# Yaling-Li/DMA-YOLO

Measured on AMD Instinct MI355X. Metric: train images/sec (fwd+loss+bwd+optimizer, train.py batch loop) @1536; detect p50 ms incl. NMS, higher is better.
Workload: dtype bf16; 1 GPU; yolov5l-ca-sppfcspc-bifpn-scconv.yaml train @1536 nc=10; model=yolov5l-ca-sppfcspc-bifpn-scconv.yaml, global_batch=32, img=1536, parallelism=dp1

## Files before the change

dma-yolo_amd/csrc/bwd1x1.hip:

```cpp
#include "common.h"

namespace {
namespace b1 {

constexpr unsigned kOob = 0xFFFFFFF0u;

DEV __amdgpu_buffer_rsrc_t rsrc(const void* base, unsigned bytes) {
  return __builtin_amdgcn_make_buffer_rsrc(const_cast<void*>(base), 0, (int)bytes, 0x00020000);
}
DEV uint4 bload(__amdgpu_buffer_rsrc_t r, unsigned off) {
  const auto v = __builtin_amdgcn_raw_buffer_load_b128(r, off, 0, 0);
  return *reinterpret_cast<const uint4*>(&v);
}

template <int ROW> DEV int ksw(int k, int row) {
  constexpr int RB = ROW * 2;
  const int c = row >> 3, w = row & 7;
  int key;
  if constexpr (RB >= 256) key = 2 * ((k & 3) | (((k >> 3) & 1) << 2));
  else key = 2 * (((k >> 1) & 1) | (((k >> 3) & 1) << 1));
  return k * ROW + (((c ^ key) & (ROW / 8 - 1)) << 3) + w;
}
template <int K> DEV int wsw(int r, int ch) {
  if constexpr (K * 2 >= 256) return (ch ^ (r & 15)) & (K / 8 - 1);
  else return (ch ^ ((r >> 1) & 7)) & (K / 8 - 1);
}
template <int ROW> DEV bf16x8 frag_t(const bf16* base, int r0, int k0, int lane) {
  typedef short s4 __attribute__((ext_vector_type(4)));
  const int g = lane >> 4, il = lane & 15, q = il >> 2, p = il & 3;
  const bf16* a0 = base + ksw<ROW>(k0 + 8 * g + q, r0 + 4 * p);
  const bf16* a1 = base + ksw<ROW>(k0 + 8 * g + 4 + q, r0 + 4 * p);
  const s4 lo = __builtin_amdgcn_ds_read_tr16_b64_v4i16((__attribute__((address_space(3))) s4*)(a0));
  const s4 hi = __builtin_amdgcn_ds_read_tr16_b64_v4i16((__attribute__((address_space(3))) s4*)(a1));
  bf16x8 r;
  r[0] = lo[0]; r[1] = lo[1]; r[2] = lo[2]; r[3] = lo[3];
  r[4] = hi[0]; r[5] = hi[1]; r[6] = hi[2]; r[7] = hi[3];
  return r;
}
DEV unsigned pk2(float a, float b) {
  const bf16 x = __float2bfloat16(a), y = __float2bfloat16(b);
  return (unsigned)*reinterpret_cast<const unsigned short*>(&x) |
         ((unsigned)*reinterpret_cast<const unsigned short*>(&y) << 16);
}

template <int K, int CB, int TP, int PX>
struct Shape {
  static constexpr int NT = 256, KCH = K / 8, CCH = CB / 8;
  static constexpr int NDZ = TP * KCH / NT, NX = TP * CCH / NT;
  static constexpr int RDZ = NT / KCH, RXS = NT / CCH;
  static constexpr int KW = K / 2, CW = CB / 2, MI = KW / 16, NJ = CW / 16;
  static constexpr int PGN = TP / (16 * PX), U = PGN * (CB / 64), UPW = (U + 3) / 4;
  static constexpr int LDS = (CB * K + TP * K + TP * CB) * 2;
  static_assert(K % 64 == 0 && CB % 64 == 0 && NT % KCH == 0 && NT % CCH == 0, "channels");
  static_assert(NDZ >= 1 && NX >= 1 && TP % 32 == 0 && TP % (16 * PX) == 0 && U >= 1, "tile");
  static_assert(LDS <= 160 * 1024, "LDS");
};

template <int K, int CB, int TP, int PX>
__global__ void __launch_bounds__(256, 1) conv1x1_bwd_bn(
    const bf16* __restrict__ dy, long dps, const bf16* __restrict__ z, const bf16* __restrict__ x, long xps,
    const bf16* __restrict__ wt, const float* __restrict__ scale, const float* __restrict__ shift,
    const float* __restrict__ mean, const float* __restrict__ invstd, int act, const float* __restrict__ ca,
    const float* __restrict__ cb, const float* __restrict__ cc, bf16* __restrict__ dx, long bps, int accumulate,
    float* __restrict__ dw, float* __restrict__ dws, long M, int ntiles, int C, int nsplit, unsigned dyb, unsigned zb,
    unsigned xb) {
  using S = Shape<K, CB, TP, PX>;
  extern __shared__ __attribute__((aligned(16))) char b1_smem[];
  bf16* ws = reinterpret_cast<bf16*>(b1_smem);
  bf16* dzs = ws + CB * K;
  bf16* xs = dzs + TP * K;
  const int tid = threadIdx.x, lane = tid & 63, wid = tid >> 6, g = lane >> 4, il = lane & 15;
  const int slot = blockIdx.x >> 3, cs = slot % nsplit;
  const int grp = (blockIdx.x & 7) + 8 * (slot / nsplit), ngrp = gridDim.x / nsplit;
  const int cbase = cs * CB;
  x += cbase;
  dx += cbase;
  dw += cbase;

  for (int e = tid; e < CB * S::KCH; e += S::NT) {
    const int r = e / S::KCH, ch = e % S::KCH;
    *reinterpret_cast<uint4*>(ws + r * K + (wsw<K>(r, ch) << 3)) =
        *reinterpret_cast<const uint4*>(wt + (long)(cbase + r) * K + ch * 8);
  }

  const int kc8 = (tid % S::KCH) * 8, xc8 = (tid % S::CCH) * 8;
  float sc[8], sh[8], k1[8], k0[8], k2[8];
  {
    float t0[8], t1[8];
    ldf<8>(scale + kc8, sc);
    ldf<8>(shift + kc8, sh);
    ldf<8>(ca + kc8, k1);
    ldf<8>(cc + kc8, k2);
    ldf<8>(invstd + kc8, t0);
    ldf<8>(cb + kc8, k0);
    ldf<8>(mean + kc8, t1);
#pragma unroll
    for (int j = 0; j < 8; ++j) {
      k2[j] = k2[j] * t0[j];
      k0[j] = k0[j] - k2[j] * t1[j];
    }
  }

  const __amdgpu_buffer_rsrc_t rdy = rsrc(dy, dyb), rz = rsrc(z, zb), rx = rsrc(x, xb - 2u * cbase);
  uint4 pg[S::NDZ], pz[S::NDZ], pxv[S::NX];
  auto issue = [&](int t) {
    const long m0 = (long)t * TP;
#pragma unroll
    for (int j = 0; j < S::NDZ; ++j) {
      const long m = m0 + tid / S::KCH + j * S::RDZ;
      const bool ok = m < M;
      pg[j] = bload(rdy, ok ? (unsigned)((m * dps + kc8) * 2) : kOob);
      pz[j] = bload(rz, ok ? (unsigned)((m * K + kc8) * 2) : kOob);
    }
#pragma unroll
    for (int j = 0; j < S::NX; ++j) {
      const long m = m0 + tid / S::CCH + j * S::RXS;
      pxv[j] = bload(rx, m < M ? (unsigned)((m * xps + xc8) * 2) : kOob);
    }
  };

  f32x4 wacc[S::MI][S::NJ];
#pragma unroll
  for (int i = 0; i < S::MI; ++i)
#pragma unroll
    for (int j = 0; j < S::NJ; ++j) wacc[i][j] = f32x4{0.f, 0.f, 0.f, 0.f};
  const int wk = wid >> 1, wc = wid & 1;
  const int chq = (g & 1) * 16 + (g >> 1) * 8;

  int t = grp;
  if (t < ntiles) issue(t);
  __syncthreads();
  for (; t < ntiles; t += ngrp) {
    const long m0 = (long)t * TP;
#pragma unroll
    for (int j = 0; j < S::NDZ; ++j) {
      float zf[8], gf[8], o[8];
      unpack<bf16>(pz[j], zf);
      unpack<bf16>(pg[j], gf);
#pragma unroll
      for (int e = 0; e < 8; ++e) o[e] = zf[e] * sc[e] + sh[e];
      act_grad_n<8>(act, o);
#pragma unroll
      for (int e = 0; e < 8; ++e) o[e] = k1[e] * (gf[e] * o[e]) + k0[e] + k2[e] * zf[e];
      pg[j] = pack<bf16>(o);
    }
    __syncthreads();
#pragma unroll
    for (int j = 0; j < S::NDZ; ++j)
      *reinterpret_cast<uint4*>(dzs + ksw<K>(tid / S::KCH + j * S::RDZ, kc8)) = pg[j];
#pragma unroll
    for (int j = 0; j < S::NX; ++j)
      *reinterpret_cast<uint4*>(xs + ksw<CB>(tid / S::CCH + j * S::RXS, xc8)) = pxv[j];
    __syncthreads();

    uint4 old[S::UPW][PX][2];
    if (accumulate) {
#pragma unroll
      for (int s = 0; s < S::UPW; ++s) {
        const int u = wid + 4 * s, p0 = (u % S::PGN) * 16 * PX, c0 = (u / S::PGN) * 64;
        if (u >= S::U) break;
#pragma unroll
        for (int pt = 0; pt < PX; ++pt) {
          const long m = m0 + p0 + pt * 16 + il;
#pragma unroll
          for (int h = 0; h < 2; ++h)
            old[s][pt][h] = m < M ? *reinterpret_cast<const uint4*>(dx + m * bps + c0 + h * 32 + chq)
                                  : make_uint4(0, 0, 0, 0);
        }
      }
    }
    if (t + ngrp < ntiles) issue(t + ngrp);

#pragma unroll
    for (int s = 0; s < S::UPW; ++s) {
      const int u = wid + 4 * s, p0 = (u % S::PGN) * 16 * PX, c0 = (u / S::PGN) * 64;
      if (u >= S::U) break;
      f32x4 acc[4][PX];
#pragma unroll
      for (int ct = 0; ct < 4; ++ct)
#pragma unroll
        for (int pt = 0; pt < PX; ++pt) acc[ct][pt] = f32x4{0.f, 0.f, 0.f, 0.f};
#pragma unroll 2
// ... 22 lines not shown
          uint4 v;
          v.x = s0[0];
          v.y = s1[0];
          v.z = s0[1];
          v.w = s1[1];
          if (accumulate) {
            float f[8], o[8];
            unpack<bf16>(v, f);
            unpack<bf16>(old[s][pt][h], o);
#pragma unroll
            for (int j = 0; j < 8; ++j) f[j] += o[j];
            v = pack<bf16>(f);
          }
          if (m < M) *reinterpret_cast<uint4*>(dx + m * bps + c0 + h * 32 + chq) = v;
        }
      }
    }

#pragma unroll
    for (int ps = 0; ps < TP / 32; ++ps) {
      bf16x8 a[S::MI];
#pragma unroll
      for (int i = 0; i < S::MI; ++i) a[i] = frag_t<K>(dzs, wk * S::KW + i * 16, ps * 32, lane);
#pragma unroll
      for (int j = 0; j < S::NJ; ++j) {
        const bf16x8 b = frag_t<CB>(xs, wc * S::CW + j * 16, ps * 32, lane);
#pragma unroll
        for (int i = 0; i < S::MI; ++i)
          wacc[i][j] = __builtin_amdgcn_mfma_f32_16x16x32_bf16(a[i], b, wacc[i][j], 0, 0, 0);
      }
    }
  }
  float* part = dws != nullptr ? dws + (long)blockIdx.x * K * CB : nullptr;
#pragma unroll
  for (int i = 0; i < S::MI; ++i)
#pragma unroll
    for (int j = 0; j < S::NJ; ++j)
#pragma unroll
      for (int r = 0; r < 4; ++r) {
        const int kk = wk * S::KW + i * 16 + 4 * g + r, c = wc * S::CW + j * 16 + il;
        if (part != nullptr) part[kk * CB + c] = wacc[i][j][r];
        else atomicAdd(dw + (long)kk * C + c, wacc[i][j][r]);
      }
}

__global__ void __launch_bounds__(256) wgrad_slots_reduce(const float* __restrict__ dws, float* __restrict__ dw, int K,
                                                          int C, int CB, int nblocks, int nsplit) {
  const long e = (long)blockIdx.x * blockDim.x + threadIdx.x;
  if (e >= (long)K * C) return;
  const int k = (int)(e / C), c = (int)(e % C), cs = c / CB, cl = c % CB;
  float s = 0.f;
  for (int b = 0; b < nblocks; ++b)
    if (((b >> 3) % nsplit) == cs) s += dws[((long)b * K + k) * CB + cl];
  dw[e] += s;
}

int num_cus() {
  static int n = 0;
  if (n == 0) {
    int dev = 0;
    (void)hipGetDevice(&dev);
    if (hipDeviceGetAttribute(&n, hipDeviceAttributeMultiprocessorCount, dev) != hipSuccess || n <= 0) n = 256;
  }
  return n;
}

struct Plan {
  int cb, tp, px;
};
constexpr Plan plan(int K, int C) {
  return (K == 64 && C == 64) ? Plan{64, 128, 2} : (K == 128 && C == 64) ? Plan{64, 128, 2}
       : (K == 64 && C == 128) ? Plan{128, 64, 2} : (K == 128 && C == 128) ? Plan{128, 64, 2}
       : (K == 128 && C == 256) ? Plan{256, 64, 2} : (K == 128 && C == 512) ? Plan{256, 64, 2}
       : (K == 256 && C == 256) ? Plan{128, 32, 1} : (K == 256 && C == 128) ? Plan{128, 32, 1}
       : (K == 64 && C == 256) ? Plan{256, 64, 2} : Plan{0, 0, 0};
}

inline int grid_blocks(long M, int K, int C) {
  const Plan pl = plan(K, C);
  const int ns = C / pl.cb, ntiles = ceil_div(M, pl.tp);
  int ngrp = num_cus() / ns;
  if (ngrp > ntiles) ngrp = (ntiles + 7) / 8 * 8;
  return ngrp * ns;
}

template <int K, int C>
int launch(const bf16* dy, long dps, const bf16* z, const bf16* x, long xps, const bf16* wt, const float* scale,
           const float* shift, const float* mean, const float* invstd, int act, const float* ca, const float* cb,
           const float* cc, bf16* dx, long bps, int acc, float* dw, float* ws, long M, hipStream_t st) {
  constexpr Plan pl = plan(K, C);
  constexpr int CB = pl.cb, TP = pl.tp, PX = pl.px, NS = C / CB;
  using S = Shape<K, CB, TP, PX>;
  static bool raised = false;
  if (!raised) {
    (void)hipFuncSetAttribute((const void*)conv1x1_bwd_bn<K, CB, TP, PX>,
                              hipFuncAttributeMaxDynamicSharedMemorySize, S::LDS);
    raised = true;
  }
  const int nb = grid_blocks(M, K, C);
  conv1x1_bwd_bn<K, CB, TP, PX><<<nb, 256, S::LDS, st>>>(
      dy, dps, z, x, xps, wt, scale, shift, mean, invstd, act, ca, cb, cc, dx, bps, acc, dw, ws, M, ceil_div(M, TP), C,
      NS, (unsigned)(2.0 * (double)M * dps), (unsigned)(2.0 * (double)M * K), (unsigned)(2.0 * (double)M * xps));
  if (ws != nullptr)
    wgrad_slots_reduce<<<ceil_div((long)K * C, 256), 256, 0, st>>>(ws, dw, K, C, CB, nb, NS);
  return (int)hipGetLastError();
}
}
}

DMY_API int dmy_conv1x1_bwd_bn_ok(long M, int K, int C, long dps, long xps, long bps, const void* dy, const void* z,
                                  const void* x, const void* dx) {
  if (b1::plan(K, C).cb == 0 || M <= 0) return 0;
  if (dps % 8 || xps % 8 || bps % 8 || dps < K || xps < C || bps < C) return 0;
  for (const void* p : {dy, z, x, dx})
    if (((uintptr_t)p & 15) != 0) return 0;
  const double lim = (double)b1::kOob - 64.0;
  if (2.0 * (double)M * dps >= lim || 2.0 * (double)M * K >= lim || 2.0 * (double)M * xps >= lim) return 0;
  return 1;
}

DMY_API long dmy_conv1x1_bwd_bn_ws_elems(long M, int K, int C) {
  if (b1::plan(K, C).cb == 0 || M <= 0) return 0;
  return (long)b1::grid_blocks(M, K, C) * K * b1::plan(K, C).cb;
}

DMY_API int dmy_conv1x1_bwd_bn(const void* dy, long dps, const void* z, const void* x, long xps, const void* wt,
                               const float* scale, const float* shift, const float* mean, const float* invstd, int act,
                               const float* ca, const float* cb, const float* cc, void* dx, long bps, int accumulate,
                               float* dw, float* ws, long ws_elems, long M, int K, int C, void* stream) {
  if (!dmy_conv1x1_bwd_bn_ok(M, K, C, dps, xps, bps, dy, z, x, dx)) return -1;
  if (ws != nullptr && ws_elems < dmy_conv1x1_bwd_bn_ws_elems(M, K, C)) return -1;
  hipStream_t st = (hipStream_t)stream;
#define B1_GO(K_, C_)                                                                                                 \
  if (K == K_ && C == C_)                                                                                            \
    return b1::launch<K_, C_>((const bf16*)dy, dps, (const bf16*)z, (const bf16*)x, xps, (const bf16*)wt, scale,     \
                              shift, mean, invstd, act, ca, cb, cc, (bf16*)dx, bps, accumulate, dw, ws, M, st);
  B1_GO(64, 64)
  B1_GO(128, 64)
  B1_GO(64, 128)
  B1_GO(128, 128)
  B1_GO(128, 256)
  B1_GO(128, 512)
  B1_GO(256, 128)
  B1_GO(256, 256)
  B1_GO(64, 256)
#undef B1_GO
  return -1;
}
```

dma-yolo_amd/dmayolo/_lib.py:

```python
import ctypes
import os

import torch

_HERE = os.path.dirname(os.path.abspath(__file__))
LIB_PATH = os.path.join(_HERE, 'libdmayolo_hip.so')
if os.environ.get('DMY_LIB_AB'):
    LIB_PATH = os.path.join(_HERE, os.path.basename(os.environ['DMY_LIB_AB']))

P, I, L, F, D = ctypes.c_void_p, ctypes.c_int, ctypes.c_long, ctypes.c_float, ctypes.c_double

SIGNATURES = {
    'dmy_conv_fwd_partial_rows': [L, I],
    'dmy_conv_fwd_bound_rows': [L, I],
    'dmy_conv_fwd_last_rows': [],
    'dmy_conv_fwd_bn_rows': [I, P, P, P, P, I, I, I, I, L, I, I, I, I, I, I, I, L],
    'dmy_conv_fwd': [I, P, P, P, P, P, P, I, I, I, I, L, I, I, I, I, I, I, I, L, P],
    'dmy_conv_dgrad': [I, P, P, P, I, I, I, I, I, L, I, I, I, I, I, I, I, L, P],
    'dmy_conv_wgrad': [I, P, P, P, I, I, I, I, L, I, I, I, I, I, I, I, L, P],
    'dmy_conv_wprep_multi': [I, P, I, P],
    'dmy_conv_wprep_s2d': [I, P, P, I, I, I, P],
    'dmy_conv_wgrad_s2d_to_oihw': [P, P, I, I, I, P],
    'dmy_image_s2d': [I, I, P, P, I, I, I, I, I, F, P],
    'dmy_conv_fwd_act': [I, P, P, P, P, I, I, I, I, L, I, I, I, I, I, I, I, L, P, P, I, P, L, P],
    'dmy_conv_fwd_splitk_elems': [I, P, P, P, I, I, I, I, L, I, I, I, I, I, I, I, L],
    'dmy_conv_fwd_act_ws': [I, P, P, P, P, I, I, I, I, L, I, I, I, I, I, I, I, L, P, P, I, P, L, P, L, P],
    'dmy_conv_wgrad_ex': [I, P, P, P, I, I, I, I, L, I, I, I, I, I, I, I, L, I, P],
    'dmy_conv_wgrad_ws_elems': [I, P, P, I, I, I, I, L, I, I, I, I, I, I, I, L, I],
    'dmy_conv_wgrad_det': [I, P, P, P, I, I, I, I, L, I, I, I, I, I, I, I, L, I, P, L, P],
    'dmy_conv_route': [I, I, P, P, P, I, I, I, I, L, I, I, I, I, I, I, I, L, I],
    'dmy_conv_wprep': [I, P, P, P, I, I, I, I, I, P],
    'dmy_dwconv_ok': [I, P, P, P, I, I, I, I, I, I, L, I, I, I, I, I, I, L],
    'dmy_dwconv_fwd_rows': [L, I],
    'dmy_dwconv_fwd': [I, P, P, P, P, P, P, I, I, I, I, L, I, I, I, I, I, I, L, P],
    'dmy_dwconv_fwd_act': [I, P, P, P, P, I, I, I, I, L, I, I, I, I, I, I, L, P, P, I, P, L, P],
    'dmy_dwconv_dgrad': [I, P, P, P, I, I, I, I, I, L, I, I, I, I, I, I, L, P],
    'dmy_dwconv_wgrad_rows': [L, I],
    'dmy_dwconv_wgrad': [I, P, P, P, I, I, I, I, L, I, I, I, I, I, I, L, P],
    'dmy_dwconv_wgrad_finalize': [P, I, I, I, I, P, I, P],
    'dmy_conv1x1_bwd_bn_ok': [L, I, I, L, L, L, P, P, P, P],
    'dmy_conv1x1_bwd_bn': [P, L, P, P, L, P, P, P, P, P, I, P, P, P, P, L, I, P, P, L, L, I, I, P],
    'dmy_conv1x1_bwd_bn_ws_elems': [L, I, I],
    'dmy_aug_desc_bytes': [],
    'dmy_augment_batch': [P, I, P, I, I, P],
    'dmy_mosaic_desc_bytes': [],
    'dmy_mosaic_compose': [P, I, I, P],
    'dmy_fp8_quant_ws_elems': [],
    'dmy_fp8_quant': [P, L, I, L, P, P, P],
    'dmy_conv_wprep_fp8': [P, P, P, I, I, I, I, P],
    'dmy_conv_fwd_fp8_partial_rows': [L, I],
    'dmy_conv_fwd_fp8': [P, P, P, P, P, P, P, P, I, I, I, I, I, I, I, I, I, I, I, L, P, P, I, P, L, P],
    'dmy_conv_wgrad_to_oihw': [P, P, I, I, I, I, I, P],
    'dmy_bn_partial_rows': [L],
    'dmy_bn_stats': [I, P, L, L, I, P, P, P],
    'dmy_bn_finalize': [P, P, I, I, D, P, P, P, P, P, F, F, I, P, P, P, P, P],
    'dmy_bn_eval_coef': [P, P, P, P, F, I, P, P, P],
    'dmy_bn_act_fwd': [I, P, L, P, P, I, P, L, P, L, L, I, P],
    'dmy_bn_act_f8_blocks': [],
    'dmy_bn_act_fwd_f8': [P, L, P, P, I, P, L, P, L, L, I, P, P, P, P, F, P, P],
    'dmy_bn_bwd_reduce': [I, P, L, P, L, P, P, P, P, I, L, I, P, P, P],
    'dmy_bn_bwd_finalize': [P, P, I, I, D, P, P, P, P, P, P, P, P],
    'dmy_bn_bwd_apply': [I, P, L, P, L, P, P, P, P, I, P, P, P, P, L, L, I, P],
    'dmy_reduce_rows': [P, I, I, P, I, P],
    'dmy_bn_reduce_rows': [I, P, L, P, L, L, I],
    'dmy_colsum2_rows': [L],
    'dmy_colsum2': [P, P, L, I, P, P, P],
    'dmy_maxpool_fwd': [I, P, L, P, L, P, I, I, I, I, I, P],
    'dmy_maxpool_chain3_fwd': [I, P, L, P, P, P, L, I, I, I, I, I, P],
    'dmy_maxpool_bwd': [I, P, L, P, P, L, I, I, I, I, I, I, P],
    'dmy_avgpool_fwd': [I, P, L, P, I, I, I, I, I, P],
    'dmy_avgpool_bwd': [I, P, P, L, I, I, I, I, I, I, P],
    'dmy_resize_fwd': [I, P, L, P, L, F, I, I, I, I, I, I, P],
    'dmy_resize_bwd': [I, P, L, P, L, I, I, I, I, I, I, P],
    'dmy_slice_copy': [I, P, L, P, L, L, I, P, I, I, F, I, P],
    'dmy_slice_copy_dot': [I, P, L, P, L, P, L, L, I, P, I, I, F, I, P, P],
# ... 123 lines not shown
```

dma-yolo_amd/dmayolo/functional.py:

```python
import os
import weakref
from collections import namedtuple

import torch

from . import _lib
from ._lib import call, ptr, stream, ACT_NONE, ACT_SILU, ACT_HARDSWISH, ACT_SIGMOID, ACT_GELU, ACT_RELU

DT = {torch.float32: 0, torch.bfloat16: 1}
CL = torch.channels_last


def dcode(t):
    try:
        return DT[t.dtype]
    except KeyError:
        raise TypeError(f'dmayolo kernels take float32 or bfloat16 activations, got {t.dtype}')


def pixel_stride(t):
    N, C, H, W = t.shape
    for attempt in range(2):
        s = t.stride()
        if C == 1 or s[1] == 1:
# ... 518 lines not shown
    if OH < 1 or OW < 1 or C % VW[x.dtype] or p != k // 2 or k not in (3, 5) or s not in (1, 2):
        raise _dw_unsupported(G, C, K, k, s, p)
    g = ConvGeom(N, C, H, W, xps, K, k, s, p, OH, OW, N * OH * OW, C, H, W, k, s, p, C, 0, G)
    w = spec.wcache[1] if infer and spec.wcache is not None and spec.wcache[0] == wkey else None
    pre = WeightPrep.current.get(weight, x.dtype) if WeightPrep.current is not None else None
    if w is None and pre is not None:
        w = pre[1]
    elif w is None:
        w = prep_weight(weight, x.dtype, True)[1]
        if infer:
            spec.wcache = (wkey, w)
    return x, g, w, w, wkey


def _conv_fp8(x, g, weight, spec, wkey, f8in, prod, infer):
    if not (spec.fp8 and g.groups == 1 and not g.s2d and g.Cp == g.C and fp8_eligible(g.C, g.K, x.dtype, g.N * g.H * g.W)):
        return None
    if f8in is not None and (f8in[0].numel() != g.N * g.H * g.W * g.C or not F8_DELAYED[0]):
        f8in = None
    f8 = _fp8_operands(x, g.xps, weight, spec, wkey, f8in)
    if f8in is None and prod is not None and prod.f8_emit is None and F8_DELAYED[0] and not infer:
        prod.f8_emit = F8Emit(x.device)
    return f8


def _conv_infer(x, g, wf, bias, spec, res, rps, out, yps, f8):
    y = out if out is not None else new_act(g.N, g.K, g.OH, g.OW, x)
    scale, shift = eval_coef(spec, x.device) if spec.bn is not None else (None, None)
    epi = None if (scale is None and spec.act == ACT_NONE and res is None) else (scale, shift, spec.act, res, rps)
    _launch_conv_fwd(x, g, wf, bias, y, yps, None, None, epi=epi, f8=f8)
    return y


def _conv_bn_stats(x, g, wf, bias, z, bn, train_bn, f8):
    K, M, dev = g.K, g.M, x.device
    scale, shift, mean, invstd = f32(K, dev), f32(K, dev), f32(K, dev), f32(K, dev)
    if not train_bn:
        _launch_conv_fwd(x, g, wf, bias, z, K, None, None, f8=f8)
        call('dmy_bn_eval_coef', ptr(bn.weight), ptr(bn.bias), ptr(bn.running_mean), ptr(bn.running_var),
             float(bn.eps), K, ptr(scale), ptr(shift), stream())
        return scale, shift, mean, invstd
    dw = g.groups != 1
    P = call('dmy_dwconv_fwd_rows' if dw else 'dmy_conv_fwd_fp8_partial_rows' if f8 is not None else
             'dmy_conv_fwd_bound_rows', M, K)
    psum, psq = f32(P * K, dev), f32(P * K, dev)
    _launch_conv_fwd(x, g, wf, bias, z, K, psum, psq, f8=f8)
    if f8 is None and not dw:
        P = call('dmy_conv_fwd_last_rows')
    psum, psq, P = _fold_partials(psum, psq, P, K, dev)
    upd = int(bn.training and bn.track_running_stats)
    if upd:
        PARAM_GEN[0] += 1
    mom = bn.momentum if bn.momentum is not None else 0.0
    call('dmy_bn_finalize', ptr(psum), ptr(psq), P, K, float(M), ptr(bn.weight), ptr(bn.bias),
         ptr(bn.running_mean) if upd else None, ptr(bn.running_var) if upd else None,
         ptr(bn.num_batches_tracked) if upd else None, float(mom), float(bn.eps), upd,
         ptr(mean), ptr(invstd), ptr(scale), ptr(shift), stream())
    return scale, shift, mean, invstd


def _defer_affine(z, stats, act, K):
    link = BnLink(*stats, act, K)
    z._dmy_affine, z._dmy_bnlink = stats, link
    return link


def _act_pass(g, z, scale, shift, spec, res, rps, out, yps, emit_ok):
    K, M = g.K, g.M
    y = out if out is not None else new_act(g.N, K, g.OH, g.OW, z)
    emit = spec.f8_emit if (emit_ok and F8_DELAYED[0] and z.dtype == torch.bfloat16 and K % 8 == 0 and yps % 8 == 0 and
                            (res is None or rps % 8 == 0)) else None
    if emit is not None and not torch.cuda.is_current_stream_capturing():
        e8 = emit.run(z, scale, shift, spec.act, res, rps, y, yps, M, K)
        if e8 is not None:
            y._dmy_f8 = e8
    else:
        call('dmy_bn_act_fwd', dcode(z), ptr(z), K, ptr(scale), ptr(shift), spec.act, ptr(res), rps, ptr(y), yps, M, K,
             stream())
    return y


def _save_ctx(ctx, saved, g, spec, train_bn, bnlink, weight, bias, gamma, beta, has_res, xsink, rsink):
    ctx.save_for_backward(*saved)
    ctx.g, ctx.spec, ctx.train_bn, ctx.bnlink = g, spec, train_bn, bnlink
    ctx.has_bias, ctx.has_res, ctx.xsink, ctx.rsink = bias is not None, has_res, xsink, rsink
    ctx.arena, ctx.wkey = WgradArena.current, weight.data_ptr()
    ctx.pkeys = tuple(t.data_ptr() if t is not None else None for t in (bias, gamma, beta))


def _pgrad(ctx, i, K, dev, zero=False):
    key = ctx.pkeys[i]
    g = ctx.arena.take(key, (K,)) if (ctx.arena is not None and key is not None) else None
    return g if g is not None else torch.zeros(K, dtype=torch.float32, device=dev) if zero else f32(K, dev)


def _wgrad_target(ctx, shape, dev):
    dw = ctx.arena.take(ctx.wkey, shape) if ctx.arena is not None else None
    return (dw, True) if dw is not None else (torch.empty(shape, dtype=torch.float32, device=dev), False)


def _bn_bwd_coef(ctx, dt, dy, dps, z, stats, gamma):
    K, M, dev = ctx.g.K, ctx.g.M, dy.device
    ca, cb, cc = f32(K, dev), f32(K, dev), f32(K, dev)
    if not ctx.train_bn:
        ca.copy_(stats[0])
        cb.zero_()
        cc.zero_()
        return ca, cb, cc, None, None
    link, rd = ctx.bnlink, None
    if link is not None:
        rd, link.ready = link.ready, None
    if rd is not None and rd[0].data_ptr() == dy.data_ptr() and rd[1] == dps and rd[0]._version == rd[5]:
        _, _, pdb, pdg, P, _ = rd
    else:
        P = call('dmy_bn_reduce_rows', dt, ptr(z), K, ptr(dy), dps, M, K)
        pdb, pdg = f32(P * K, dev), f32(P * K, dev)
        call('dmy_bn_bwd_reduce', dt, ptr(z), K, ptr(dy), dps, *map(ptr, stats), ctx.spec.act, M, K, ptr(pdb),
             ptr(pdg), stream())
    pdb, pdg, P = _fold_partials(pdb, pdg, P, K, dev)
    dgamma, dbeta = _pgrad(ctx, 1, K, dev), _pgrad(ctx, 2, K, dev)
    call('dmy_bn_bwd_finalize', ptr(pdb), ptr(pdg), P, K, float(M), ptr(gamma), ptr(stats[3]), ptr(dgamma), ptr(dbeta),
         ptr(ca), ptr(cb), ptr(cc), stream())
    return ca, cb, cc, dgamma, dbeta


def _bwd1x1(ctx, dy, dps, x, wt, z, stats, coef):
    g = ctx.g
    N, C, H, W, xps, K, M = g.N, g.C, g.H, g.W, g.xps, g.K, g.M
    if not (BWD1X1[0] and g.groups == 1 and ctx.train_bn and g.k == 1 and g.s == 1 and g.p == 0 and not g.s2d and g.Cp == C and
            dy.dtype == torch.bfloat16 and wt is not None and ctx.needs_input_grad[0] and ctx.needs_input_grad[1]):
        return None
    buf_probe = ctx.xsink.peek(N, C, H, W) if ctx.xsink is not None else None
    bps_probe = buf_probe[1] if buf_probe is not None else C
    if not call('dmy_conv1x1_bwd_bn_ok', M, K, C, dps, xps, bps_probe, ptr(dy), ptr(z), ptr(x),
                ptr(buf_probe[0]) if buf_probe is not None else ptr(z)):
        return None
# ... 104 lines not shown
            else:
                y = _act_pass(g, z, stats[0], stats[1], spec, res, rps, out, yps, True)
                if x.dtype == torch.bfloat16 and g.K % 128 == 0 and train_bn:
                    y._dmy_prod = spec
        _save_ctx(ctx, saved, g, spec, train_bn, link, weight, bias, gamma, beta, res is not None, xsink, rsink)
        return y

    @staticmethod
    def backward(ctx, dy):
        g, spec = ctx.g, ctx.spec
        x, wt, z, *bnt = ctx.saved_tensors
        dy, dps = pixel_stride(dy.to(z.dtype))
        K, dev, dt = g.K, dy.device, dcode(dy)
        dbias = dgamma = dbeta = fused = None
        if spec.bn is not None:
            *stats, gamma = bnt
            *coef, dgamma, dbeta = _bn_bwd_coef(ctx, dt, dy, dps, z, stats, gamma)
            fused = _bwd1x1(ctx, dy, dps, x, wt, z, stats, coef)
            if fused is None:
                dz, dzps = new_act(g.N, K, g.OH, g.OW, z), K
                call('dmy_bn_bwd_apply', dt, ptr(z), K, ptr(dy), dps, *map(ptr, stats), spec.act, *map(ptr, coef),
                     ptr(dz), K, g.M, K, stream())
            if ctx.has_bias and ctx.train_bn:
                dbias = _pgrad(ctx, 0, K, dev, zero=True)
        else:
            dz, dzps, dbias = _act_bias_bwd(ctx, dt, dy, dps, z)
        if fused is not None:
            dx, dw = fused
        else:
            dx = _dgrad(ctx, dt, dz, dzps, wt, z) if ctx.needs_input_grad[0] else None
            dw = _conv_wgrad(ctx, dt, x, dz, dzps) if ctx.needs_input_grad[1] else None
        dres = (dy if ctx.rsink is None else ctx.rsink.passthrough(dy)) if ctx.has_res else None
        return dx, dw, dbias, dgamma, dbeta, dres, None, None, None, None, None


def conv_bn_act(x, weight, bias, bn, stride, pad, act, res=None, spec=None, xsink=None, rsink=None, out=None,
                defer=False):
    if spec is None:
        spec = _param_spec(weight._base if weight._base is not None else weight, stride, pad, act, bn)
    spec.defer = bool(defer)
    gamma = bn.weight if bn is not None else None
    beta = bn.bias if bn is not None else None
    return ConvBNActFn.apply(x, weight, bias, gamma, beta, res, spec, xsink, rsink, torch.is_grad_enabled(),
                             [out] if out is not None else None)



class MaxPoolFn(torch.autograd.Function):
    @staticmethod
    def forward(ctx, x, k, sink=None, out=None):
        x, xps = pixel_stride(x)
        N, C, H, W = x.shape
        y, yps = out_view(out and out[0], (N, C, H, W), x)
        if y is None:
            y, yps = new_act(N, C, H, W, x), C
        arg = torch.empty((N, H, W, C), dtype=torch.uint8, device=x.device)
        call('dmy_maxpool_fwd', dcode(x), ptr(x), xps, ptr(y), yps, ptr(arg), N, H, W, C, k, stream())
        ctx.save_for_backward(arg)
        ctx.k, ctx.shape, ctx.sink = k, (N, C, H, W), sink
        return y

    @staticmethod
    def backward(ctx, dy):
        (arg,) = ctx.saved_tensors
        N, C, H, W = ctx.shape
        dy, dps = pixel_stride(dy)
# ... 663 lines not shown
```

dma-yolo_amd/dmayolo/models/common.py:

```python
import math
import os
import weakref

import torch
import torch.nn as nn

from .. import functional as Fn
from ..functional import ACT_NONE, ACT_SILU, ACT_HARDSWISH, ACT_SIGMOID, ACT_GELU, ACT_RELU

__all__ = ['autopad', 'Conv', 'DWConv', 'GhostConv', 'GhostBottleneck', 'C3Ghost', 'Bottleneck', 'C3', 'SPPF', 'SPPFCSPC', 'SCConv', 'CoorAttention', 'CA',
           'CABottleneck', 'C3CA', 'Concat', 'AdConcat2', 'AdConcat3', 'Upsample', 'C3STR', 'SwinTransformerBlock',
           'SwinTransformerLayer', 'WindowAttention', 'Mlp', 'DropPath', 'space_to_depth', 'SPP', 'CBAM',
           'ChannelAttentionModule', 'SpatialAttentionModule', 'C3TR', 'TransformerBlock', 'TransformerLayer']


def autopad(k, p=None):
    if p is None:
        p = k // 2 if isinstance(k, int) else [x // 2 for x in k]
    return p


def act_code(m):
    if m is None or isinstance(m, nn.Identity):
        return ACT_NONE
# ... 129 lines not shown
    def _pair(self):
        c1, c2 = self.cv1, self.cv2
        b1, b2 = getattr(c1, 'bn', None), getattr(c2, 'bn', None)
        w1, w2 = c1.conv.weight, c2.conv.weight
        if (b1 is None) != (b2 is None) or type(c1.act) is not type(c2.act) or w1.shape[1:] != w2.shape[1:] or \
                tuple(w1.shape[2:]) != (1, 1) or tuple(c1.conv.stride) != (1, 1) or tuple(c2.conv.stride) != (1, 1) or \
                (b1 is not None and (b1.eps != b2.eps or b1.training or b2.training)) or \
                (c1.conv.bias is None) != (c2.conv.bias is None):
            return None
        srcs = [w1, w2, c1.conv.bias, c2.conv.bias] + ([b1.weight, b1.bias, b1.running_mean, b1.running_var, b2.weight,
                                                        b2.bias, b2.running_mean, b2.running_var] if b1 is not None else [])
        key = (Fn.PARAM_GEN[0],) + tuple((t.data_ptr(), t._version) if t is not None else None for t in srcs)
        ent = _PAIRS.get(self)
        if ent is None or ent[0] != key:
            w = torch.cat([w1.detach(), w2.detach()])
            b = torch.cat([c1.conv.bias.detach(), c2.conv.bias.detach()]) if c1.conv.bias is not None else None
            ent = _PAIRS[self] = (key, w, b, _PairBN(b1, b2) if b1 is not None else None, act_code(c1.act))
        return ent[1:]

    def forward(self, x, out=None):
        blocks = list(self.m) if isinstance(self.m, nn.Sequential) else []
        seq = bool(blocks) and type(blocks[-1]) is Bottleneck and _INPLACE_CAT >= 1
        pair = self._pair() if seq and _C3_PAIR and not self.training and not torch.is_grad_enabled() else None
        if pair is not None:
            w, b, bn, act = pair
            c_ = w.shape[0] // 2
            cat = Fn.concat_buffer(x.shape[0], 2 * c_, x.shape[2], x.shape[3], x)
            Fn.conv_bn_act(x, w, b, bn, 1, 0, act, out=cat)
            a = cat[:, :c_]
            for blk in blocks[:-1]:
                a = blk(a)
            a = blocks[-1](a, out=cat[:, :c_])
            return self.cv3(Fn.ConcatFn.apply(None, 0.0, None, a, cat[:, c_:]), out=out)
        sk = Fn.GradSink(2)
        a = self.cv1(x, xsink=sk)
        if not seq and not (getattr(self.m, 'dmy_out', False) and _INPLACE_CAT >= 2):
            return self.cv3(Fn.ConcatFn.apply(None, 0.0, None, self.m(a), self.cv2(x, xsink=sk)), out=out)
        c_ = a.shape[1]
        cat = Fn.concat_buffer(a.shape[0], 2 * c_, a.shape[2], a.shape[3], a)
        if seq:
            for b in blocks[:-1]:
                a = b(a)
            a = blocks[-1](a, out=cat[:, :c_])
        else:
            a = self.m(a, out=cat[:, :c_])
        return self.cv3(Fn.ConcatFn.apply(None, 0.0, None, a, self.cv2(x, xsink=sk, out=cat[:, c_:])), out=out)


class C3Ghost(C3):

    def __init__(self, c1, c2, n=1, shortcut=True, g=1, e=0.5):
        super().__init__(c1, c2, n, shortcut, g, e)
        c_ = int(c2 * e)
        self.m = nn.Sequential(*(GhostBottleneck(c_, c_) for _ in range(n)))


class SPPF(nn.Module):

    def __init__(self, c1, c2, k=5):
        super().__init__()
        c_ = c1 // 2
        self.cv1 = Conv(c1, c_, 1, 1)
        self.cv2 = Conv(c_ * 4, c2, 1, 1)
        self.m = nn.MaxPool2d(kernel_size=k, stride=1, padding=k // 2)

    def forward(self, x):
        k = self.m.kernel_size
        c_ = self.cv1.conv.out_channels
        if _INPLACE_CAT >= 1:
            cat = Fn.concat_buffer(x.shape[0], 4 * c_, x.shape[2], x.shape[3], x)
            sl = [cat[:, i * c_:(i + 1) * c_] for i in range(4)]
        else:
            sl = [None] * 4
        x = self.cv1(x, out=sl[0])
        ys = Fn.maxpool_chain3(x, k, sl[1:])
        if ys is not None:
            return self.cv2(Fn.ConcatFn.apply(None, 0.0, None, x, *ys))
        s0, s1, s2 = Fn.GradSink(2), Fn.GradSink(2), Fn.GradSink(2)
        y1 = Fn.MaxPoolFn.apply(x, k, s0, sl[1:2])
# ... 329 lines not shown
```

include/dmayolo.h:

```cpp
#ifndef DMAYOLO_H
#define DMAYOLO_H
#ifdef __cplusplus
extern "C" {
#endif

int dmy_conv_fwd_partial_rows(long M, int K);
long dmy_conv_fwd_bound_rows(long M, int K);
long dmy_conv_fwd_last_rows(void);
int dmy_conv_fwd_bn_rows(int dtype, const void* x, const void* w_ohwi, const float* bias, const void* y, int N,
                                int H, int W, int C, long xps, int K, int KH, int KW, int S, int P, int OH, int OW,
                                long yps);
int dmy_conv_fwd(int dtype, const void* x, const void* w_ohwi, const float* bias, void* y, float* psum, float* psq,
                 int N, int H, int W, int C, long xps, int K, int KH, int KW, int S, int P, int OH, int OW, long yps,
                 void* stream);
int dmy_conv_fwd_act(int dtype, const void* x, const void* w_ohwi, const float* bias, void* y, int N, int H, int W,
                     int C, long xps, int K, int KH, int KW, int S, int P, int OH, int OW, long yps, const float* scale,
                     const float* shift, int act, const void* res, long rps, void* stream);
long dmy_conv_fwd_splitk_elems(int dtype, const void* x, const void* w_ohwi, const void* y, int N, int H, int W, int C,
                               long xps, int K, int KH, int KW, int S, int P, int OH, int OW, long yps);
int dmy_conv_fwd_act_ws(int dtype, const void* x, const void* w_ohwi, const float* bias, void* y, int N, int H, int W,
                        int C, long xps, int K, int KH, int KW, int S, int P, int OH, int OW, long yps, const float* scale,
                        const float* shift, int act, const void* res, long rps, float* ws, long ws_elems, void* stream);
int dmy_conv_dgrad(int dtype, const void* dy, const void* w_ihwo, void* dx, int accumulate, int N, int H, int W, int C,
                   long xps, int K, int KH, int KW, int S, int P, int OH, int OW, long yps, void* stream);
int dmy_conv_wgrad(int dtype, const void* x, const void* dy, float* dw_ohwi, int N, int H, int W, int C, long xps,
                   int K, int KH, int KW, int S, int P, int OH, int OW, long yps, void* stream);
int dmy_conv1x1_bwd_bn_ok(long M, int K, int C, long dps, long xps, long bps, const void* dy, const void* z,
                          const void* x, const void* dx);
int dmy_conv1x1_bwd_bn(const void* dy, long dps, const void* z, const void* x, long xps, const void* wt,
                       const float* scale, const float* shift, const float* mean, const float* invstd, int act,
                       const float* ca, const float* cb, const float* cc, void* dx, long bps, int accumulate,
                       float* dw, float* ws, long ws_elems, long M, int K, int C, void* stream);
long dmy_conv1x1_bwd_bn_ws_elems(long M, int K, int C);
int dmy_conv_wgrad_ex(int dtype, const void* x, const void* dy, float* dw, int N, int H, int W, int C, long xps, int K,
                      int KH, int KW, int S, int P, int OH, int OW, long yps, int flags, void* stream);
long dmy_conv_wgrad_ws_elems(int dtype, const void* x, const void* dy, int N, int H, int W, int C, long xps, int K,
                             int KH, int KW, int S, int P, int OH, int OW, long yps, int flags);
int dmy_conv_wgrad_det(int dtype, const void* x, const void* dy, float* dw, int N, int H, int W, int C, long xps,
                       int K, int KH, int KW, int S, int P, int OH, int OW, long yps, int flags, float* ws,
                       long ws_elems, void* stream);
int dmy_conv_route(int pass, int dtype, const void* a, const void* b, const void* c, int N, int H, int W, int C,
                   long xps, int K, int KH, int KW, int S, int P, int OH, int OW, long yps, int acc);
enum {
  DMY_KERN_HALO = 0,
  DMY_KERN_SPLITK = 1,
  DMY_KERN_P1S = 2,
  DMY_KERN_STEM = 3,
  DMY_KERN_P1P = 4,
  DMY_KERN_PIPE8 = 5,
  DMY_KERN_WIDE = 6,
  DMY_KERN_WIDE288 = 7,
  DMY_KERN_TALL = 8,
  DMY_KERN_V3 = 9,
  DMY_KERN_V2 = 10,
  DMY_KERN_V2_BIG = 11,
  DMY_KERN_S2_Q2S = 12,
  DMY_KERN_S2_Q2 = 13,
  DMY_KERN_S2_MERGED = 14,
  DMY_KERN_S2_CLASS = 15,
  DMY_KERN_W_TAP128 = 16,
  DMY_KERN_W_TAP64 = 17,
  DMY_KERN_W_TAP64X2 = 18,
  DMY_KERN_W_V4 = 19,
  DMY_KERN_W_V3 = 20,
  DMY_KERN_W_V3N128 = 21,
  DMY_KERN_W_V3N256 = 22,
// ... 239 lines not shown
```

Measured before the change: 162.1 images/s.

## Fuse C3 cv1/cv2 1x1 conv backward into one stacked-K paired kernel

Adds a PAIR mode to the fused 1x1 conv+BN backward kernel. The two sibling 1x1 convs in a C3 block (cv1 and cv2, which share input x) are handled as one stacked conv with 2K output channels: each half of the block loads its own dy/z, and the weight gradients are written to two separate buffers. The aim is to read x once, produce dx in one pass without a second accumulate pass, and save kernel launches. Forward runs through a new autograd function that keeps BN stats in contiguous stacked buffers, and there is a fallback to the split path. This adds code complexity, and the new half-block chunk mapping needs a matching plan per (K,C) shape.

```diff
diff --git a/dma-yolo_amd/csrc/bwd1x1.hip b/dma-yolo_amd/csrc/bwd1x1.hip
--- a/dma-yolo_amd/csrc/bwd1x1.hip
+++ b/dma-yolo_amd/csrc/bwd1x1.hip
@@ -56,15 +56,28 @@
   static_assert(LDS <= 160 * 1024, "LDS");
 };
 
-template <int K, int CB, int TP, int PX>
+struct Second {
+  const bf16* dy;
+  long dps;
+  const bf16* z;
+  const bf16* wt;
+  float* dw;
+  unsigned dyb;
+};
+template <int K, int CB, int TP, int PX, bool PAIR = false>
 __global__ void __launch_bounds__(256, 1) conv1x1_bwd_bn(
     const bf16* __restrict__ dy, long dps, const bf16* __restrict__ z, const bf16* __restrict__ x, long xps,
     const bf16* __restrict__ wt, const float* __restrict__ scale, const float* __restrict__ shift,
     const float* __restrict__ mean, const float* __restrict__ invstd, int act, const float* __restrict__ ca,
     const float* __restrict__ cb, const float* __restrict__ cc, bf16* __restrict__ dx, long bps, int accumulate,
     float* __restrict__ dw, float* __restrict__ dws, long M, int ntiles, int C, int nsplit, unsigned dyb, unsigned zb,
-    unsigned xb) {
+    unsigned xb, Second sec) {
   using S = Shape<K, CB, TP, PX>;
+  constexpr int KL = PAIR ? K / 2 : K;
+  constexpr int LCH = KL / 8;
+  constexpr int LNT = PAIR ? 128 : S::NT;
+  constexpr int RDZ = LNT / LCH;
+  static_assert(!PAIR || (LNT % LCH == 0 && TP % RDZ == 0 && TP / RDZ == S::NDZ), "pair chunk map");
   extern __shared__ __attribute__((aligned(16))) char b1_smem[];
   bf16* ws = reinterpret_cast<bf16*>(b1_smem);
   bf16* dzs = ws + CB * K;
@@ -76,14 +89,22 @@
   x += cbase;
   dx += cbase;
   dw += cbase;
+  const int half = PAIR ? __builtin_amdgcn_readfirstlane(tid >> 7) : 0;
+  if constexpr (PAIR) {
+    sec.dw += cbase;
+    if (half) dy = sec.dy, dps = sec.dps, z = sec.z, dyb = sec.dyb;
+  }
 
   for (int e = tid; e < CB * S::KCH; e += S::NT) {
     const int r = e / S::KCH, ch = e % S::KCH;
-    *reinterpret_cast<uint4*>(ws + r * K + (wsw<K>(r, ch) << 3)) =
-        *reinterpret_cast<const uint4*>(wt + (long)(cbase + r) * K + ch * 8);
-  }
-
-  const int kc8 = (tid % S::KCH) * 8, xc8 = (tid % S::CCH) * 8;
+    const bf16* src = wt + (long)(cbase + r) * KL + ch * 8;
+    if constexpr (PAIR)
+      if (ch >= LCH) src = sec.wt + (long)(cbase + r) * KL + (ch - LCH) * 8;
+    *reinterpret_cast<uint4*>(ws + r * K + (wsw<K>(r, ch) << 3)) = *reinterpret_cast<const uint4*>(src);
+  }
+
+  const int ltid = PAIR ? (tid & 127) : tid;
+  const int zc8 = (ltid % LCH) * 8, kc8 = half * KL + zc8, prow = ltid / LCH, xc8 = (tid % S::CCH) * 8;
   float sc[8], sh[8], k1[8], k0[8], k2[8];
   {
     float t0[8], t1[8];
@@ -107,10 +128,10 @@
     const long m0 = (long)t * TP;
 #pragma unroll
     for (int j = 0; j < S::NDZ; ++j) {
-      const long m = m0 + tid / S::KCH + j * S::RDZ;
+      const long m = m0 + prow + j * RDZ;
       const bool ok = m < M;
-      pg[j] = bload(rdy, ok ? (unsigned)((m * dps + kc8) * 2) : kOob);
-      pz[j] = bload(rz, ok ? (unsigned)((m * K + kc8) * 2) : kOob);
+      pg[j] = bload(rdy, ok ? (unsigned)((m * dps + zc8) * 2) : kOob);
+      pz[j] = bload(rz, ok ? (unsigned)((m * KL + zc8) * 2) : kOob);
     }
 #pragma unroll
     for (int j = 0; j < S::NX; ++j) {
@@ -147,7 +168,7 @@
     __syncthreads();
 #pragma unroll
     for (int j = 0; j < S::NDZ; ++j)
-      *reinterpret_cast<uint4*>(dzs + ksw<K>(tid / S::KCH + j * S::RDZ, kc8)) = pg[j];
+      *reinterpret_cast<uint4*>(dzs + ksw<K>(prow + j * RDZ, kc8)) = pg[j];
 #pragma unroll
     for (int j = 0; j < S::NX; ++j)
       *reinterpret_cast<uint4*>(xs + ksw<CB>(tid / S::CCH + j * S::RXS, xc8)) = pxv[j];
@@ -236,6 +257,10 @@
     }
   }
   float* part = dws != nullptr ? dws + (long)blockIdx.x * K * CB : nullptr;
+  float* dwl = dw;
+  int kl0 = wk * S::KW;
+  if constexpr (PAIR)
+    if (wk) dwl = sec.dw, kl0 = 0;
 #pragma unroll
   for (int i = 0; i < S::MI; ++i)
 #pragma unroll
@@ -244,19 +269,21 @@
       for (int r = 0; r < 4; ++r) {
         const int kk = wk * S::KW + i * 16 + 4 * g + r, c = wc * S::CW + j * 16 + il;
         if (part != nullptr) part[kk * CB + c] = wacc[i][j][r];
-        else atomicAdd(dw + (long)kk * C + c, wacc[i][j][r]);
+        else atomicAdd(dwl + (long)(kl0 + i * 16 + 4 * g + r) * C + c, wacc[i][j][r]);
       }
 }
 
 __global__ void __launch_bounds__(256) wgrad_slots_reduce(const float* __restrict__ dws, float* __restrict__ dw, int K,
-                                                          int C, int CB, int nblocks, int nsplit) {
+                                                          int C, int CB, int nblocks, int nsplit,
+                                                          float* __restrict__ dw2 = nullptr) {
   const long e = (long)blockIdx.x * blockDim.x + threadIdx.x;
   if (e >= (long)K * C) return;
   const int k = (int)(e / C), c = (int)(e % C), cs = c / CB, cl = c % CB;
   float s = 0.f;
   for (int b = 0; b < nblocks; ++b)
     if (((b >> 3) % nsplit) == cs) s += dws[((long)b * K + k) * CB + cl];
-  dw[e] += s;
+  if (dw2 != nullptr && k >= K / 2) dw2[e - (long)(K / 2) * C] += s;
+  else dw[e] += s;
 }
 
 int num_cus() {
@@ -280,6 +307,10 @@
        : (K == 64 && C == 256) ? Plan{256, 64, 2} : Plan{0, 0, 0};
 }
 
+constexpr bool pair_plan(int K, int C) {
+  return (K == 64 && C == 64) || (K == 128 && C == 128) || (K == 128 && C == 256) || (K == 256 && C == 256);
+}
+
 inline int grid_blocks(long M, int K, int C) {
   const Plan pl = plan(K, C);
   const int ns = C / pl.cb, ntiles = ceil_div(M, pl.tp);
@@ -288,25 +319,28 @@
   return ngrp * ns;
 }
 
-template <int K, int C>
+template <int K, int C, bool PAIR = false>
 int launch(const bf16* dy, long dps, const bf16* z, const bf16* x, long xps, const bf16* wt, const float* scale,
            const float* shift, const float* mean, const float* invstd, int act, const float* ca, const float* cb,
-           const float* cc, bf16* dx, long bps, int acc, float* dw, float* ws, long M, hipStream_t st) {
+           const float* cc, bf16* dx, long bps, int acc, float* dw, float* ws, long M, hipStream_t st,
+           Second sec = Second{}) {
   constexpr Plan pl = plan(K, C);
   constexpr int CB = pl.cb, TP = pl.tp, PX = pl.px, NS = C / CB;
   using S = Shape<K, CB, TP, PX>;
   static bool raised = false;
   if (!raised) {
-    (void)hipFuncSetAttribute((const void*)conv1x1_bwd_bn<K, CB, TP, PX>,
+    (void)hipFuncSetAttribute((const void*)conv1x1_bwd_bn<K, CB, TP, PX, PAIR>,
                               hipFuncAttributeMaxDynamicSharedMemorySize, S::LDS);
     raised = true;
   }
   const int nb = grid_blocks(M, K, C);
-  conv1x1_bwd_bn<K, CB, TP, PX><<<nb, 256, S::LDS, st>>>(
+  constexpr int KL = PAIR ? K / 2 : K;
+  sec.dyb = (unsigned)(2.0 * (double)M * sec.dps);
+  conv1x1_bwd_bn<K, CB, TP, PX, PAIR><<<nb, 256, S::LDS, st>>>(
       dy, dps, z, x, xps, wt, scale, shift, mean, invstd, act, ca, cb, cc, dx, bps, acc, dw, ws, M, ceil_div(M, TP), C,
-      NS, (unsigned)(2.0 * (double)M * dps), (unsigned)(2.0 * (double)M * K), (unsigned)(2.0 * (double)M * xps));
+      NS, (unsigned)(2.0 * (double)M * dps), (unsigned)(2.0 * (double)M * KL), (unsigned)(2.0 * (double)M * xps), sec);
   if (ws != nullptr)
-    wgrad_slots_reduce<<<ceil_div((long)K * C, 256), 256, 0, st>>>(ws, dw, K, C, CB, nb, NS);
+    wgrad_slots_reduce<<<ceil_div((long)K * C, 256), 256, 0, st>>>(ws, dw, K, C, CB, nb, NS, PAIR ? sec.dw : nullptr);
   return (int)hipGetLastError();
 }
 }
@@ -351,3 +385,39 @@
 #undef B1_GO
   return -1;
 }
+
+DMY_API int dmy_conv1x1_bwd_bn_pair_ok(long M, int K, int C, long dps, long dps2, long xps, long bps, const void* dy,
+                                       const void* dy2, const void* z, const void* z2, const void* x, const void* dx) {
+  if (!b1::pair_plan(K, C)) return 0;
+  const int KL = K / 2;
+  if (M <= 0 || dps % 8 || dps2 % 8 || xps % 8 || bps % 8 || dps < KL || dps2 < KL || xps < C || bps < C) return 0;
+  for (const void* p : {dy, dy2, z, z2, x, dx})
+    if (((uintptr_t)p & 15) != 0) return 0;
+  const double lim = (double)b1::kOob - 64.0;
+  if (2.0 * (double)M * dps >= lim || 2.0 * (double)M * dps2 >= lim || 2.0 * (double)M * KL >= lim ||
+      2.0 * (double)M * xps >= lim)
+    return 0;
+  return 1;
+}
+
+DMY_API int dmy_conv1x1_bwd_bn_pair(const void* dy, long dps, const void* z, const void* wt, float* dw, const void* dy2,
+                                    long dps2, const void* z2, const void* wt2, float* dw2, const void* x, long xps,
+                                    const float* scale, const float* shift, const float* mean, const float* invstd,
+                                    int act, const float* ca, const float* cb, const float* cc, void* dx, long bps,
+                                    int accumulate, float* ws, long ws_elems, long M, int K, int C, void* stream) {
+  if (!dmy_conv1x1_bwd_bn_pair_ok(M, K, C, dps, dps2, xps, bps, dy, dy2, z, z2, x, dx)) return -1;
+  if (ws != nullptr && ws_elems < dmy_conv1x1_bwd_bn_ws_elems(M, K, C)) return -1;
+  hipStream_t st = (hipStream_t)stream;
+  const b1::Second sec{(const bf16*)dy2, dps2, (const bf16*)z2, (const bf16*)wt2, dw2, 0u};
+#define B1_PAIR(K_, C_)                                                                                              \
+  if (K == K_ && C == C_)                                                                                            \
+    return b1::launch<K_, C_, true>((const bf16*)dy, dps, (const bf16*)z, (const bf16*)x, xps, (const bf16*)wt,      \
+                                    scale, shift, mean, invstd, act, ca, cb, cc, (bf16*)dx, bps, accumulate, dw, ws, \
+                                    M, st, sec);
+  B1_PAIR(64, 64)
+  B1_PAIR(128, 128)
+  B1_PAIR(128, 256)
+  B1_PAIR(256, 256)
+#undef B1_PAIR
+  return -1;
+}
diff --git a/dma-yolo_amd/dmayolo/_lib.py b/dma-yolo_amd/dmayolo/_lib.py
--- a/dma-yolo_amd/dmayolo/_lib.py
+++ b/dma-yolo_amd/dmayolo/_lib.py
@@ -41,6 +41,8 @@
     'dmy_conv1x1_bwd_bn_ok': [L, I, I, L, L, L, P, P, P, P],
     'dmy_conv1x1_bwd_bn': [P, L, P, P, L, P, P, P, P, P, I, P, P, P, P, L, I, P, P, L, L, I, I, P],
     'dmy_conv1x1_bwd_bn_ws_elems': [L, I, I],
+    'dmy_conv1x1_bwd_bn_pair_ok': [L, I, I, L, L, L, L, P, P, P, P, P, P],
+    'dmy_conv1x1_bwd_bn_pair': [P, L, P, P, P, P, L, P, P, P, P, L, P, P, P, P, I, P, P, P, P, L, I, P, L, L, I, I, P],
     'dmy_aug_desc_bytes': [],
     'dmy_augment_batch': [P, I, P, I, I, P],
     'dmy_mosaic_desc_bytes': [],
diff --git a/dma-yolo_amd/dmayolo/functional.py b/dma-yolo_amd/dmayolo/functional.py
--- a/dma-yolo_amd/dmayolo/functional.py
+++ b/dma-yolo_amd/dmayolo/functional.py
@@ -574,9 +574,9 @@
     return y
 
 
-def _conv_bn_stats(x, g, wf, bias, z, bn, train_bn, f8):
+def _conv_bn_stats(x, g, wf, bias, z, bn, train_bn, f8, bufs=None):
     K, M, dev = g.K, g.M, x.device
-    scale, shift, mean, invstd = f32(K, dev), f32(K, dev), f32(K, dev), f32(K, dev)
+    scale, shift, mean, invstd = bufs if bufs is not None else (f32(K, dev), f32(K, dev), f32(K, dev), f32(K, dev))
     if not train_bn:
         _launch_conv_fwd(x, g, wf, bias, z, K, None, None, f8=f8)
         call('dmy_bn_eval_coef', ptr(bn.weight), ptr(bn.bias), ptr(bn.running_mean), ptr(bn.running_var),
@@ -641,9 +641,9 @@
     return (dw, True) if dw is not None else (torch.empty(shape, dtype=torch.float32, device=dev), False)
 
 
-def _bn_bwd_coef(ctx, dt, dy, dps, z, stats, gamma):
+def _bn_bwd_coef(ctx, dt, dy, dps, z, stats, gamma, bufs=None):
     K, M, dev = ctx.g.K, ctx.g.M, dy.device
-    ca, cb, cc = f32(K, dev), f32(K, dev), f32(K, dev)
+    ca, cb, cc = bufs if bufs is not None else (f32(K, dev), f32(K, dev), f32(K, dev))
     if not ctx.train_bn:
         ca.copy_(stats[0])
         cb.zero_()
@@ -814,6 +814,122 @@
             dw = _conv_wgrad(ctx, dt, x, dz, dzps) if ctx.needs_input_grad[1] else None
         dres = (dy if ctx.rsink is None else ctx.rsink.passthrough(dy)) if ctx.has_res else None
         return dx, dw, dbias, dgamma, dbeta, dres, None, None, None, None, None
+
+
+PAIR_BWD = [os.environ.get('DMY_C3_PAIR_BWD', '1') == '1']
+PAIR_COUNT = {'fwd': 0, 'bwd_stacked': 0, 'bwd_split': 0}
+
+
+class _LayerCtx:
+
+    def __init__(self, g, spec, weight, gamma, beta, arena, needs):
+        self.g, self.spec, self.train_bn, self.bnlink = g, spec, True, None
+        self.has_bias, self.has_res, self.xsink, self.rsink = False, False, None, None
+        self.arena, self.wkey = arena, weight.data_ptr()
+        self.pkeys = (None, gamma.data_ptr(), beta.data_ptr())
+        self.needs_input_grad = needs
+
+
+def pair_eligible(x, c1, b1, a1, c2, b2, a2):
+    w1, w2 = c1.weight, c2.weight
+    return (PAIR_BWD[0] and BWD1X1[0] and b1 is not None and b2 is not None and b1.training and b2.training and
+            b1.eps == b2.eps and a1 == a2 and c1.bias is None and c2.bias is None and w1.shape == w2.shape and
+            tuple(w1.shape[2:]) == (1, 1) and tuple(c1.stride) == (1, 1) and tuple(c2.stride) == (1, 1) and
+            _pad_of(c1) == 0 and _pad_of(c2) == 0 and c1.groups == 1 and c2.groups == 1 and
+            x.dtype == torch.bfloat16 and x.dim() == 4 and torch.is_grad_enabled() and x.requires_grad and
+            w1.requires_grad and w2.requires_grad and not getattr(c1, 'dmy_fp8', False) and
+            not getattr(c2, 'dmy_fp8', False) and not getattr(x, '_dmy_s2d', 0) and
+            bool(call('dmy_conv1x1_bwd_bn_pair_ok', x.shape[0] * x.shape[2] * x.shape[3], 2 * w1.shape[0], w1.shape[1],
+                      w1.shape[0], w1.shape[0], w1.shape[1], w1.shape[1], None, None, None, None, None, None)))
+
+
+def _pad_of(conv):
+    return conv.padding if isinstance(conv.padding, int) else conv.padding[0]
+
+
+class ConvPairFn(torch.autograd.Function):
+
+    @staticmethod
+    def forward(ctx, x, w1, g1, b1, w2, g2, b2, spec1, spec2, out2=None):
+        dev = x.device
+        ws, saved, ys, subs = (w1, w2), [], [], []
+        K = w1.shape[0]
+        st4 = [f32(2 * K, dev) for _ in range(4)]
+        x0 = x
+        for i, (w, gamma, beta, spec, out) in enumerate(((w1, g1, b1, spec1, None), (w2, g2, b2, spec2, out2))):
+            x, g, wf, wt, _ = _conv_operands(x0, w, spec, True, False)
+            out, yps = out_view(out and out[0], (g.N, g.K, g.OH, g.OW), x)
+            yps = g.K if out is None else yps
+            z = new_act(g.N, g.K, g.OH, g.OW, x)
+            stats = _conv_bn_stats(x, g, wf, None, z, spec.bn, True, None,
+                                   bufs=tuple(t[i * K:(i + 1) * K] for t in st4))
+            y = _act_pass(g, z, stats[0], stats[1], spec, None, 0, out, yps, True)
+            if g.K % 128 == 0:
+                y._dmy_prod = spec
+            saved += [wt, z, gamma]
+            ys.append(y)
+            subs.append(_LayerCtx(g, spec, w, gamma, beta, WgradArena.current, (True, True)))
+        ctx.save_for_backward(x, *st4, *saved)
+        ctx.subs = subs
+        PAIR_COUNT['fwd'] += 1
+        return ys[0], ys[1]
+
+    @staticmethod
+    def backward(ctx, dy1, dy2):
+        x, *rest = ctx.saved_tensors
+        st4, (wt1, z1, gm1, wt2, z2, gm2) = rest[:4], rest[4:]
+        s1, s2 = ctx.subs
+        g = s1.g
+        N, C, H, W, xps, K, M = g.N, g.C, g.H, g.W, g.xps, g.K, g.M
+        dev, dt = x.device, dcode(z1)
+        co3 = [f32(2 * K, dev) for _ in range(3)]
+        lay = []
+        for i, (sub, dy, z, gm) in enumerate(((s1, dy1, z1, gm1), (s2, dy2, z2, gm2))):
+            dy, dps = pixel_stride(dy.to(z.dtype))
+            stats = tuple(t[i * K:(i + 1) * K] for t in st4)
+            *coef, dgamma, dbeta = _bn_bwd_coef(sub, dt, dy, dps, z, stats, gm,
+                                                bufs=tuple(t[i * K:(i + 1) * K] for t in co3))
+            lay.append((dy, dps, stats, coef, dgamma, dbeta))
+        (dya, dpa), (dyb, dpb) = lay[0][:2], lay[1][:2]
+        if PAIR_BWD[0] and wt1 is not None and wt2 is not None and call(
+                'dmy_conv1x1_bwd_bn_pair_ok', M, 2 * K, C, dpa, dpb, xps, C, ptr(dya), ptr(dyb), ptr(z1), ptr(z2),
+                ptr(x), ptr(z1)):
+            dx = new_act(N, C, H, W, z1)
+            dws = []
+            for sub in (s1, s2):
+                dw, zeroed = _wgrad_target(sub, (K, C, 1, 1), dev)
+                if not zeroed:
+                    dw.zero_()
+                dws.append(dw)
+            ne = call('dmy_conv1x1_bwd_bn_ws_elems', M, 2 * K, C) if DETERMINISTIC[0] else 0
+            ws = f32(ne, dev) if ne else None
+            KernelTimer.run('conv_bwd1x1', 8.0 * M * K * C, 'dmy_conv1x1_bwd_bn_pair', ptr(dya), dpa, ptr(z1), ptr(wt1),
+                            ptr(dws[0]), ptr(dyb), dpb, ptr(z2), ptr(wt2), ptr(dws[1]), ptr(x), xps, *map(ptr, st4),
+                            s1.spec.act, *map(ptr, co3), ptr(dx), C, 0, ptr(ws), ne, M, 2 * K, C, stream(),
+                            tag=g.tag(), nbytes=z1.element_size() * (4 * M * K + 2 * M * C + 2 * K * C) + 8 * K * C)
+            PAIR_COUNT['bwd_stacked'] += 1
+        else:
+            sk, dws, dx = GradSink(2), [None, None], None
+            for i, (sub, wt, z) in ((1, (s2, wt2, z2)), (0, (s1, wt1, z1))):
+                dy, dps, stats, coef = lay[i][:4]
+                sub.xsink = sk
+                fused = _bwd1x1(sub, dy, dps, x, wt, z, stats, coef)
+                if fused is None:
+                    dz = new_act(N, K, H, W, z)
+                    call('dmy_bn_bwd_apply', dt, ptr(z), K, ptr(dy), dps, *map(ptr, stats), sub.spec.act,
+                         *map(ptr, coef), ptr(dz), K, M, K, stream())
+                    fused = _dgrad(sub, dt, dz, K, wt, z), _conv_wgrad(sub, dt, x, dz, K)
+                dx, dws[i] = fused[0] if fused[0] is not None else dx, fused[1]
+                sub.xsink = None
+            PAIR_COUNT['bwd_split'] += 1
+        return dx, dws[0], lay[0][4], lay[0][5], dws[1], lay[1][4], lay[1][5], None, None, None
+
+
+def conv_pair(x, conv1, bn1, act1, conv2, bn2, act2, out2=None):
+    sp1, sp2 = spec_for(conv1, 1, 0, act1, bn1), spec_for(conv2, 1, 0, act2, bn2)
+    sp1.defer = sp2.defer = False
+    return ConvPairFn.apply(x, conv1.weight, bn1.weight, bn1.bias, conv2.weight, bn2.weight, bn2.bias, sp1, sp2,
+                            [out2] if out2 is not None else None)
 
 
 def conv_bn_act(x, weight, bias, bn, stride, pad, act, res=None, spec=None, xsink=None, rsink=None, out=None,
diff --git a/dma-yolo_amd/dmayolo/models/common.py b/dma-yolo_amd/dmayolo/models/common.py
--- a/dma-yolo_amd/dmayolo/models/common.py
+++ b/dma-yolo_amd/dmayolo/models/common.py
@@ -185,19 +185,29 @@
                 a = blk(a)
             a = blocks[-1](a, out=cat[:, :c_])
             return self.cv3(Fn.ConcatFn.apply(None, 0.0, None, a, cat[:, c_:]), out=out)
-        sk = Fn.GradSink(2)
-        a = self.cv1(x, xsink=sk)
-        if not seq and not (getattr(self.m, 'dmy_out', False) and _INPLACE_CAT >= 2):
-            return self.cv3(Fn.ConcatFn.apply(None, 0.0, None, self.m(a), self.cv2(x, xsink=sk)), out=out)
-        c_ = a.shape[1]
-        cat = Fn.concat_buffer(a.shape[0], 2 * c_, a.shape[2], a.shape[3], a)
+        inplace = seq or (getattr(self.m, 'dmy_out', False) and _INPLACE_CAT >= 2)
+        l1, l2 = self.cv1, self.cv2
+        paired = self.training and all(type(l) is Conv and getattr(l, 'bn', None) is not None for l in (l1, l2)) and \
+            Fn.pair_eligible(x, l1.conv, l1.bn, act_code(l1.act), l2.conv, l2.bn, act_code(l2.act))
+        c_ = l1.conv.out_channels
+        cat = Fn.concat_buffer(x.shape[0], 2 * c_, x.shape[2], x.shape[3], x) if inplace else None
+        if paired:
+            a, y2 = Fn.conv_pair(x, l1.conv, l1.bn, act_code(l1.act), l2.conv, l2.bn, act_code(l2.act),
+                                 out2=cat[:, c_:] if inplace else None)
+        else:
+            sk = Fn.GradSink(2)
+            a = self.cv1(x, xsink=sk)
+        if not inplace:
+            return self.cv3(Fn.ConcatFn.apply(None, 0.0, None, self.m(a),
+                                              y2 if paired else self.cv2(x, xsink=sk)), out=out)
         if seq:
             for b in blocks[:-1]:
                 a = b(a)
             a = blocks[-1](a, out=cat[:, :c_])
         else:
             a = self.m(a, out=cat[:, :c_])
-        return self.cv3(Fn.ConcatFn.apply(None, 0.0, None, a, self.cv2(x, xsink=sk, out=cat[:, c_:])), out=out)
+        return self.cv3(Fn.ConcatFn.apply(None, 0.0, None, a,
+                                          y2 if paired else self.cv2(x, xsink=sk, out=cat[:, c_:])), out=out)
 
 
 class C3Ghost(C3):
diff --git a/include/dmayolo.h b/include/dmayolo.h
--- a/include/dmayolo.h
+++ b/include/dmayolo.h
@@ -32,6 +32,13 @@
                        const float* ca, const float* cb, const float* cc, void* dx, long bps, int accumulate,
                        float* dw, float* ws, long ws_elems, long M, int K, int C, void* stream);
 long dmy_conv1x1_bwd_bn_ws_elems(long M, int K, int C);
+int dmy_conv1x1_bwd_bn_pair_ok(long M, int K, int C, long dps, long dps2, long xps, long bps, const void* dy,
+                               const void* dy2, const void* z, const void* z2, const void* x, const void* dx);
+int dmy_conv1x1_bwd_bn_pair(const void* dy, long dps, const void* z, const void* wt, float* dw, const void* dy2,
+                            long dps2, const void* z2, const void* wt2, float* dw2, const void* x, long xps,
+                            const float* scale, const float* shift, const float* mean, const float* invstd, int act,
+                            const float* ca, const float* cb, const float* cc, void* dx, long bps, int accumulate,
+                            float* ws, long ws_elems, long M, int K, int C, void* stream);
 int dmy_conv_wgrad_ex(int dtype, const void* x, const void* dy, float* dw, int N, int H, int W, int C, long xps, int K,
                       int KH, int KW, int S, int P, int OH, int OW, long yps, int flags, void* stream);
 long dmy_conv_wgrad_ws_elems(int dtype, const void* x, const void* dy, int N, int H, int W, int C, long xps, int K,
```

Measured after the change: 162.7 images/s, median of 6. About the same (+0.4%).
